# puzzlepaint/camera_calibration

Measured on NVIDIA H100. Metric: LM iterations/sec, higher is better.
Workload: dtype f64

## Files before the change

### camera_calibration_b200/build.py

```python
from __future__ import annotations

import os
import subprocess
import sys
from concurrent.futures import ThreadPoolExecutor

HERE = os.path.dirname(os.path.abspath(__file__))
CSRC = os.path.join(HERE, "csrc")
LIB = os.path.join(CSRC, "libb200ba.so")
SOURCES = ["ba_kernels.cu", "ba_host.cu", "ba_dense.cu"]
HEADERS = ["ba_common.h", "ba_device.cuh", "ba_kernels.h", os.path.join("..", "..", "include", "b200ba.h")]
NVCC = os.environ.get("NVCC", "/usr/local/cuda/bin/nvcc")
FLAGS = ["-gencode", "arch=compute_90a,code=sm_90a", "-lineinfo", "-O3", "-std=c++17", "-Xcompiler", "-fPIC",
         "-Xcompiler", "-fvisibility=hidden"]


def _stale() -> bool:
    if not os.path.exists(LIB):
        return True
    t = os.path.getmtime(LIB)
    for f in SOURCES + HEADERS:
        if os.path.getmtime(os.path.join(CSRC, f)) > t:
            return True
    return False


# ... 27 lines not shown
```

### camera_calibration_b200/csrc/ba_dense.cu

```cuda

#include <algorithm>
#include <cstdio>

#include "ba_kernels.h"
#include "ba_tile.cuh"

namespace b200ba {

namespace {

constexpr int BM = 128;
constexpr int LDT = BM + 4;
__host__ __device__ constexpr int gemm_threads(int bn) { return 4 * (bn / 32) * 32; }
constexpr size_t gemm_smem(int bn, int bk, int stages) {
  return static_cast<size_t>(stages) * bk * (LDT + bn + 4) * sizeof(double);
}

__device__ __forceinline__ void cp_async16(void* smem, const void* gmem, int src_bytes) {
  const unsigned s = static_cast<unsigned>(__cvta_generic_to_shared(smem));
  asm volatile("cp.async.cg.shared.global [%0], [%1], 16, %2;\n" ::"r"(s), "l"(gmem), "r"(src_bytes));
}
__device__ __forceinline__ void cp_async8(void* smem, const void* gmem, int src_bytes) {
  const unsigned s = static_cast<unsigned>(__cvta_generic_to_shared(smem));
  asm volatile("cp.async.ca.shared.global [%0], [%1], 8, %2;\n" ::"r"(s), "l"(gmem), "r"(src_bytes));
// ... 302 lines not shown
    configured_dev[dev & 63] = true;
  }
  potrf_trinv_tile_kernel<<<tile::CTAS, tile::THREADS, sizeof(tile::Shared), s>>>(Ain, lda_in, n, Lout, lda_out, Linv, info);
  return cudaGetLastError() == cudaSuccess ? 0 : 1;
}

__global__ void add_diagonal_map_kernel(int n, double* S, DenseMap map, double lambda) {
  const int c = blockIdx.x * blockDim.x + threadIdx.x;
  if (c < n) S[map.col_offset(c) + c] += lambda;
}
void launch_add_diagonal_map(int n, double* S, const DenseMap& map, double lambda, cudaStream_t s) {
  if (n > 0) add_diagonal_map_kernel<<<(n + 255) / 256, 256, 0, s>>>(n, S, map, lambda);
}

__global__ void trsv_store_tile_kernel(const double* __restrict__ Linv, const double* __restrict__ b, int live,
                                       double* __restrict__ out, bool transpose) {
  const int tid = threadIdx.x;
  if (tid >= live) return;
  double acc = 0.0;
  if (!transpose) {
    for (int c = 0; c <= tid; ++c) acc = fma(Linv[c * PT + tid], b[c], acc);
  } else {
    for (int i = tid; i < live; ++i) acc = fma(Linv[tid * PT + i], b[i], acc);
  }
  out[tid] = acc;
}

constexpr int TS2_THREADS = 256;
constexpr int TS2_LD = PT + 2;
constexpr size_t kTs2Smem = static_cast<size_t>(PT) * TS2_LD * sizeof(double);

__device__ __forceinline__ void stage_tile_async(double* dst, const double* __restrict__ src) {
  for (int ch = threadIdx.x; ch < PT * PT / 2; ch += TS2_THREADS) {
    const int c = ch >> 6, i2 = (ch & 63) * 2;
    cp_async16(dst + c * TS2_LD + i2, src + c * PT + i2, 16);
  }
  cp_async_commit();
}

// ... 35 lines not shown
      b_below[r] = v;
  }
  if (!chain) return;
  cp_async_wait<0>();
  __syncthreads();
  double s0 = 0.0, s1 = 0.0;
  for (int c = half; c <= row; c += 4) {
    s0 = fma(ts2_smem[c * TS2_LD + row], bs[c], s0);
    if (c + 2 <= row) s1 = fma(ts2_smem[(c + 2) * TS2_LD + row], bs[c + 2], s1);
  }
  part[half][row] = s0 + s1;
  __syncthreads();
  if (half == 0 && live_row) y_next[row] = part[0][row] + part[1][row];
}

__global__ void __launch_bounds__(TS2_THREADS, 1)
    trsv_backward2_kernel(const double* __restrict__ Lpack, const int64_t* __restrict__ panel_off,
                          const int* __restrict__ panel_h, int NB, int r0, int live, const double* __restrict__ x_t,
                          double* __restrict__ y , const double* __restrict__ Linv_prev,
                          double* __restrict__ x_prev ) {
  extern __shared__ __align__(16) double ts2_smem[];
  __shared__ double xs[PT], ysm[PT], part[2][PT];
  const int tid = threadIdx.x;
  const bool chain = blockIdx.x == 0;
  if (chain) stage_tile_async(ts2_smem, Linv_prev);
  if (tid < PT) xs[tid] = (tid < live) ? x_t[tid] : 0.0;
  __syncthreads();
  const int warp = tid >> 5, lane = tid & 31;
  const int cbase = r0 - PT * (static_cast<int>(blockIdx.x) + 1);
#pragma unroll
  for (int batch = 0; batch < 2; ++batch) {
    double l[8][4];
#pragma unroll
    for (int q = 0; q < 8; ++q) {
      const int c = cbase + warp * 16 + batch * 8 + q;
      const int k = c / NB;
      const double* col = Lpack + panel_off[k] + static_cast<int64_t>(c - k * NB) * panel_h[k] + (r0 - k * NB);
#pragma unroll
      for (int u = 0; u < 4; ++u) l[q][u] = (lane + 32 * u < live) ? col[lane + 32 * u] : 0.0;
    }
#pragma unroll
    for (int q = 0; q < 8; ++q) {
      double acc = 0.0;
#pragma unroll
      for (int u = 0; u < 4; ++u) acc = fma(l[q][u], xs[lane + 32 * u], acc);
#pragma unroll
      for (int o = 16; o > 0; o >>= 1) acc += __shfl_xor_sync(0xffffffffu, acc, o);
      if (lane == 0) {
        const int c = cbase + warp * 16 + batch * 8 + q;
        const double v = y[c] - acc;
        if (chain)
          ysm[c - cbase] = v;
        else
          y[c] = v;
      }
    }
  }
  if (!chain) return;
  cp_async_wait<0>();
  __syncthreads();
  const int j = tid & (PT - 1), half = tid >> 7;
  double s0 = 0.0, s1 = 0.0;
  const double* colj = ts2_smem + j * TS2_LD;
  for (int i = j + half; i < PT; i += 4) {
    s0 = fma(colj[i], ysm[i], s0);
    if (i + 2 < PT) s1 = fma(colj[i + 2], ysm[i + 2], s1);
  }
  part[half][j] = s0 + s1;
  __syncthreads();
  if (half == 0) x_prev[j] = part[0][j] + part[1][j];
}

int dense_plan(DenseCtx* d, int n, int nb, int rank, int ranks) {
  d->n = n;
  d->rank = rank;
  d->ranks = ranks;
  d->NB = nb;
  d->nblk = (n + nb - 1) / nb;
  d->ntiles = (n + PT - 1) / PT;
  d->map.nb = nb;
  d->map.ranks = ranks;
  d->map.blocks_per_rank = (d->nblk + ranks - 1) / ranks;
  d->map.ld = (n + 1) / 2 * 2;
  d->chunk = static_cast<int64_t>(d->map.blocks_per_rank) * nb * d->map.ld;
  d->panel_off.assign(d->nblk + 1, 0);
  d->panel_h.assign(std::max(1, d->nblk), 0);
  for (int k = 0; k < d->nblk; ++k) {
    const int hk = n - k * nb;
    d->panel_h[k] = (hk + 1) / 2 * 2;
    d->panel_off[k + 1] = d->panel_off[k] + static_cast<int64_t>(d->panel_h[k]) * nb + static_cast<int64_t>(nb / PT) * PT * PT;
  }
  return 0;
}

int dense_factor(DenseCtx* d) {
  const int n = d->n, NB = d->NB, R = d->ranks, me = d->rank;
  if (n == 0) return 0;
  const int sub_n = NB / PT;
  cudaStream_t sm = d->s_main, sp = d->s_panel;
  auto owner = [&](int k) { return k % R; };
  const bool use_aux = R == 1 && d->s_aux != nullptr;
  cudaEventRecord(d->ev_misc, sm);
  cudaStreamWaitEvent(sp, d->ev_misc, 0);

  auto update = [&](int k, int j_first, int j_last, cudaStream_t st, bool owned_only) -> int {
    if (j_first >= d->nblk || j_first > j_last) return 0;
    const int k0 = k * NB, kw = std::min(NB, n - k0);
    const int j0 = j_first * NB;
    const int jn = std::min(n, (std::min(j_last, d->nblk - 1) + 1) * NB) - j0;
    if (jn <= 0) return 0;
    GemmArgs g{};
    g.M = n - j0;
    g.N = jn;
    g.K = kw;
    g.A = d->Lpack + d->panel_off[k] + (j0 - k0);
    g.lda = d->panel_h[k];
    g.B = g.A;
    g.ldb = g.lda;
// ... 56 lines not shown
            u.ldb = hk;
            u.C = Sk_w + static_cast<int64_t>(c0 + PT) * ld + (c0 + PT);
            u.ldc = ld;
            u.alpha = -1.0;
            u.beta = 1.0;
            u.a_aligned = u.b_aligned = gemm_operand_aligned(u.A, u.lda);
            if (launch_dgemm_nt(u, true, false, sp, true)) return 1;
          }
        }
      }
    }
    if (R > 1) {
      if (d->bcast(P, static_cast<size_t>(hk) * NB + static_cast<size_t>(sub_n) * PT * PT, owner(k), sp, d->user)) return 1;
    }
    cudaEventRecord(d->ev_ready[k & 1], sp);
    cudaStreamWaitEvent(sm, d->ev_ready[k & 1], 0);
    if (k + 3 < d->nblk && update(k, k + 3, d->nblk - 1, sm, R > 1)) return 1;
    cudaEventRecord(d->ev_main[k & 1], sm);
    if (use_aux) {
      if (k >= 1) cudaStreamWaitEvent(sp, d->ev_half2[(k - 1) & 1], 0);
      if (k + 1 < d->nblk && update(k, k + 1, k + 1, sp, false)) return 1;
      if (k + 2 < d->nblk) {
        cudaStreamWaitEvent(d->s_aux, d->ev_ready[k & 1], 0);
        if (k > 0) cudaStreamWaitEvent(d->s_aux, d->ev_main[(k - 1) & 1], 0);
        if (update(k, k + 2, k + 2, d->s_aux, false)) return 1;
      }
      cudaEventRecord(d->ev_half2[k & 1], d->s_aux);
      continue;
    }
    if (k + 1 < d->nblk && owner(k + 1) == me && update(k, k + 1, k + 1, sp, false)) return 1;
    if (k + 2 < d->nblk && owner(k + 2) == me) {
      if (k > 0) cudaStreamWaitEvent(sp, d->ev_main[(k - 1) & 1], 0);
      if (update(k, k + 2, k + 2, sp, false)) return 1;
    }
  }
  if (use_aux && d->nblk >= 1) cudaStreamWaitEvent(sp, d->ev_half2[(d->nblk - 1) & 1], 0);
  cudaEventRecord(d->ev_misc, sp);
  cudaStreamWaitEvent(sm, d->ev_misc, 0);
  return cudaGetLastError() == cudaSuccess ? 0 : 1;
}

int dense_solve(DenseCtx* d, double* b) {
  const int n = d->n, NB = d->NB;
  if (n == 0) return 0;
  cudaStream_t sm = d->s_main;
  auto linv_of = [&](int t) {
    const int k = (t * PT) / NB, sub = (t * PT - k * NB) / PT;
    return d->Lpack + d->panel_off[k] + static_cast<int64_t>(d->panel_h[k]) * NB + static_cast<int64_t>(sub) * PT * PT;
  };
  static bool configured_dev[64] = {};
  int dev = 0;
  cudaGetDevice(&dev);
  if (!configured_dev[dev & 63]) {
    cudaFuncSetAttribute(trsv_forward2_kernel, cudaFuncAttributeMaxDynamicSharedMemorySize, static_cast<int>(kTs2Smem));
    cudaFuncSetAttribute(trsv_backward2_kernel, cudaFuncAttributeMaxDynamicSharedMemorySize, static_cast<int>(kTs2Smem));
    configured_dev[dev & 63] = true;
  }
  const int T = d->ntiles;
  trsv_store_tile_kernel<<<1, PT, 0, sm>>>(linv_of(0), b, std::min(PT, n), d->tmp, false);
  for (int t = 0; t + 1 < T; ++t) {
    const int c0 = t * PT, k = c0 / NB, off = c0 - k * NB;
    const int rows_below = n - c0 - PT;
    const double* Lp = d->Lpack + d->panel_off[k] + static_cast<int64_t>(off) * d->panel_h[k] + off + PT;
    trsv_forward2_kernel<<<(rows_below + PT - 1) / PT, TS2_THREADS, kTs2Smem, sm>>>(Lp, d->panel_h[k], rows_below, d->tmp + c0,
                                                                                    b + c0 + PT, linv_of(t + 1), d->tmp + c0 + PT);
  }
  {
    const int r0 = (T - 1) * PT;
    trsv_store_tile_kernel<<<1, PT, 0, sm>>>(linv_of(T - 1), d->tmp + r0, std::min(PT, n - r0), b + r0, true);
  }
  for (int t = T - 1; t >= 1; --t) {
    const int r0 = t * PT, live = std::min(PT, n - r0);
    trsv_backward2_kernel<<<r0 / PT, TS2_THREADS, kTs2Smem, sm>>>(d->Lpack, d->d_panel_off, d->d_panel_h, NB, r0, live, b + r0,
                                                                  d->tmp, linv_of(t - 1), b + r0 - PT);
  }
  return cudaGetLastError() == cudaSuccess ? 0 : 1;
}


constexpr int GV_ROWS = 128;
__global__ void gemv_t_stage1_kernel(int rows, int cols, int64_t ld, const double* __restrict__ B,
                                     const double* __restrict__ u, double* __restrict__ partial) {
  const int c = blockIdx.x * blockDim.x + threadIdx.x;
  const int r0 = blockIdx.y * GV_ROWS, r1 = min(rows, r0 + GV_ROWS);
  if (c >= cols) return;
  double a0 = 0.0, a1 = 0.0;
  int r = r0;
  for (; r + 1 < r1; r += 2) {
    a0 = fma(B[static_cast<int64_t>(r) * ld + c], u[r], a0);
    a1 = fma(B[static_cast<int64_t>(r + 1) * ld + c], u[r + 1], a1);
  }
  if (r < r1) a0 = fma(B[static_cast<int64_t>(r) * ld + c], u[r], a0);
  partial[static_cast<int64_t>(blockIdx.y) * cols + c] = a0 + a1;
// ... 42 lines not shown
```

### camera_calibration_b200/csrc/ba_host.cu

```cuda

#include <cublas_v2.h>
#include <cusolverDn.h>
#include <dlfcn.h>

#include <algorithm>
#include <cmath>
#include <cstdarg>
#include <cstdio>
#include <cstring>
#include <limits>
#include <string>
#include <vector>

#include "ba_kernels.h"

using namespace b200ba;

namespace {

std::string g_create_error;

struct NcclUniqueId {
  char internal[128];
};
// ... 124 lines not shown
  bool have_report = false;
  std::vector<int64_t> img_cam_groups;
  int* d_img_group_off = nullptr;
  uint32_t* d_img_group_obs = nullptr;
  bool have_images = false;

  void* comm = nullptr;
  int rank = 0, n_ranks = 1;

  bool own_dense = true;
  DenseCtx dn;
  int dense_planned_ranks = 0, dense_planned_n = -1;
  int dense_nb = 0;
  cudaStream_t panel_stream = nullptr;
  cudaStream_t aux_stream = nullptr;
  int* d_ident_cols = nullptr;
  double* d_gemv_partial = nullptr;

  b200ba_timings timings{};
  struct Pending {
    int phase;
    cudaEvent_t a, b;
    bool own_a = true;
  };
  std::vector<Pending> pending;
  std::vector<cudaEvent_t> event_pool;
};

namespace {

// ... 211 lines not shown
  if (rc != 0) {
    h->error = std::string("ncclBroadcast: ") + (g_nccl.GetErrorString ? g_nccl.GetErrorString(rc) : "error");
    return 1;
  }
  return 0;
}

cudaError_t dense_create(DenseCtx* d, bool own_streams) {
  cudaError_t e = cudaSuccess;
  if (own_streams) {
    int lo = 0, hi = 0;
    cudaDeviceGetStreamPriorityRange(&lo, &hi);
    e = cudaStreamCreateWithFlags(&d->s_main, cudaStreamNonBlocking);
    if (e == cudaSuccess) e = cudaStreamCreateWithPriority(&d->s_panel, cudaStreamNonBlocking, hi);
    if (e == cudaSuccess) e = cudaStreamCreateWithPriority(&d->s_aux, cudaStreamNonBlocking, hi);
  }
  for (cudaEvent_t* ev : {&d->ev_ready[0], &d->ev_ready[1], &d->ev_main[0], &d->ev_main[1], &d->ev_half2[0],
                          &d->ev_half2[1], &d->ev_misc})
    if (e == cudaSuccess && !*ev) e = cudaEventCreateWithFlags(ev, cudaEventDisableTiming);
  return e;
}
void dense_release(DenseCtx* d, bool own_streams) {
  for (cudaEvent_t ev : {d->ev_ready[0], d->ev_ready[1], d->ev_main[0], d->ev_main[1], d->ev_half2[0], d->ev_half2[1],
                         d->ev_misc})
    if (ev) cudaEventDestroy(ev);
  if (own_streams)
    for (cudaStream_t s : {d->s_main, d->s_panel, d->s_aux})
      if (s) cudaStreamDestroy(s);
}

int plan_dense(b200ba_handle* h) {
  if (!h->own_dense || !h->have_layout) return 0;
  const int nd = h->L.nd;
  if (h->dense_planned_n == nd && h->dense_planned_ranks == h->n_ranks) return 0;
  DenseCtx& d = h->dn;
  const int nb = h->dense_nb > 0 ? h->dense_nb : (h->n_ranks == 1 ? 512 : 256);
  dense_plan(&d, nd, nb, h->rank, h->n_ranks);
  if (dev_alloc(h, &h->d_S, static_cast<size_t>(std::max<int64_t>(1, d.chunk * h->n_ranks)))) return 1;
  d.S = h->d_S;
  if (dev_alloc(h, &d.Lpack, static_cast<size_t>(std::max<int64_t>(1, d.panel_off[d.nblk])))) return 1;
  if (dev_alloc(h, &d.tmp, std::max(1, nd))) return 1;
  if (dev_alloc(h, &d.d_panel_off, d.panel_off.size())) return 1;
  if (dev_alloc(h, &d.d_panel_h, d.panel_h.size())) return 1;
  CUDA_TRY(h, cudaMemcpy(d.d_panel_off, d.panel_off.data(), d.panel_off.size() * sizeof(int64_t), cudaMemcpyHostToDevice));
  CUDA_TRY(h, cudaMemcpy(d.d_panel_h, d.panel_h.data(), d.panel_h.size() * sizeof(int), cudaMemcpyHostToDevice));
  {
    std::vector<int> ident(std::max(1, nd));
    for (int i = 0; i < nd; ++i) ident[i] = i;
    if (dev_alloc(h, &h->d_ident_cols, ident.size())) return 1;
    CUDA_TRY(h, cudaMemcpy(h->d_ident_cols, ident.data(), ident.size() * sizeof(int), cudaMemcpyHostToDevice));
  }
  if (dev_alloc(h, &h->d_gemv_partial, static_cast<size_t>(gemv_t_partial_size(h->L.nbd, std::max(1, nd))))) return 1;
  CUDA_TRY(h, cudaMemset(h->d_S, 0, static_cast<size_t>(std::max<int64_t>(1, d.chunk * h->n_ranks)) * sizeof(double)));
  d.info = h->d_info;
  d.s_main = h->stream;
  d.s_panel = h->panel_stream;
  d.s_aux = h->aux_stream;
  CUDA_TRY(h, dense_create(&d, false));
  d.bcast = nccl_bcast_cb;
  d.user = h;
  h->dense_planned_n = nd;
  h->dense_planned_ranks = h->n_ranks;
  return 0;
}

int make_layout(b200ba_handle* h, const b200ba_options* opt) {
  if (opt->regularization_weight != 0) {
    static bool warned = false;
    if (!warned) fprintf(stderr, "[b200ba] regularization_weight is ignored (the term is disabled in the reference, joint_optimization.cc:299-305)\n");
    warned = true;
  }
  Layout L{};
// ... 490 lines not shown
    if (L.nbd > 0 && nd > 0) launch_gemv_t(L.nbd, nd, nd, h->sys.B, h->d_u, -1.0, h->d_x + L.nbd, h->d_gemv_partial, h->stream);
    h->timings.kernel_launches += 4;
  }
  if (h->capture_S && capture_reduced_system(h)) return 1;
  if (R > 1 && nd > 0) {
    ScopedPhase ph(h, PH_ALLREDUCE);
    const int rc = g_nccl.ReduceScatter(h->d_S, h->d_S + static_cast<size_t>(h->rank) * d.chunk, static_cast<size_t>(d.chunk),
                                        kNcclDouble, kNcclSum, h->comm, h->stream);
    if (rc != 0) {
      h->error = std::string("ncclReduceScatter: ") + (g_nccl.GetErrorString ? g_nccl.GetErrorString(rc) : "error");
      return 1;
    }
  }
  {
    ScopedPhase ph(h, PH_FACTOR);
    if (dense_factor(&d)) {
      if (h->error.empty()) h->error = "dense_factor: launch failed";
      return 1;
    }
    h->timings.factor_flops += static_cast<double>(nd) * nd * nd / 3.0;
    if (R > 1) {
      const int rc = g_nccl.AllReduce(h->d_info, h->d_info, 1, kNcclInt32, kNcclMax, h->comm, h->stream);
      if (rc != 0) {
        h->error = "ncclAllReduce (factorisation status) failed";
        return 1;
      }
    }
  }
  {
    ScopedPhase ph(h, PH_SOLVE);
    if (dense_solve(&d, h->d_x + L.nbd)) {
      h->error = "dense_solve: launch failed";
      return 1;
    }
    h->timings.kernel_launches += 4 * d.ntiles;
  }
  {
    ScopedPhase ph(h, PH_SCHUR);
    if (L.nbd > 0 && nd > 0)
      launch_gemv_n(L.nbd, nd, nd, h->sys.B, h->d_x + L.nbd, h->d_y, h->stream);
    else if (L.nbd > 0)
      CUDA_TRY(h, cudaMemsetAsync(h->d_y, 0, L.nbd * sizeof(double), h->stream));
    launch_block_backsub2(L.bs, L.nblocks, h->d_Linv, h->d_u, h->d_y, h->d_x, h->stream);
    h->timings.kernel_launches += 1;
  }
  CUDA_TRY(h, cudaMemcpyAsync(h->h_flags, h->d_info, sizeof(int), cudaMemcpyDeviceToHost, h->stream));
  CUDA_TRY(h, cudaMemcpyAsync(h->h_flags + 1, h->d_fail, sizeof(int), cudaMemcpyDeviceToHost, h->stream));
  if (sync_stream(h)) return 1;
  *spd = (h->h_flags[0] == 0 && h->h_flags[1] == 0) ? 1 : 0;
  return 0;
}

int check_ready(b200ba_handle* h, const b200ba_options* opt) {
  if (!h) return 1;
  if (!opt) {
    h->error = "options are NULL";
    return 2;
  }
  if (!h->have_state) {
    h->error = "no state: call b200ba_set_state first";
    return 2;
  }
  CUDA_TRY(h, cudaSetDevice(h->device));
// ... 17 lines not shown
  F(h->out_trial.residual); F(h->out_trial.cost);
  F(h->sys.base); F(h->d_W); F(h->d_S); F(h->d_Linv); F(h->d_v); F(h->d_y); F(h->d_x); F(h->d_potrf_work);
  F(h->d_info); F(h->d_fail); F(h->d_straggler_list); F(h->d_straggler_count); F(h->d_perm); F(h->d_lp_stage);
  F(h->d_group_of_block); F(h->d_group_blocks); F(h->d_flags); F(h->d_cols); F(h->d_count); F(h->d_Wc); F(h->d_P); F(h->d_u);
  F(h->d_contract);
  if (h->h_count) cudaFreeHost(h->h_count);
  h->h_count = nullptr;
  if (h->h_contract) cudaFreeHost(h->h_contract);
  h->h_contract = nullptr;
  F(h->d_partial); F(h->d_scal); F(h->d_rot);
  F(h->rep.err); F(h->rep.mag); F(h->rep.cam_off); F(h->rep.cell_off); F(h->rep.cell_order); F(h->rep.Q);
  F(h->rep.partial); F(h->rep.select_hist); F(h->rep.hist); F(h->rep.kl); F(h->rep.cams); F(h->d_rep_stage);
  h->have_report = false;
  F(h->d_img_group_off); F(h->d_img_group_obs);
  h->have_images = false;
  F(h->dn.Lpack); F(h->dn.tmp); F(h->dn.d_panel_off); F(h->dn.d_panel_h); F(h->d_ident_cols); F(h->d_gemv_partial);
  h->dn.S = nullptr;
  h->dense_planned_n = -1;
  if (h->h_scal) cudaFreeHost(h->h_scal);
  if (h->h_flags) cudaFreeHost(h->h_flags);
  h->h_scal = nullptr;
  h->h_flags = nullptr;
}

int setup_report(b200ba_handle* h) {
  if (h->have_report) return 0;
  const int64_t n = h->n_obs;
  const int nc = h->n_cameras;
  constexpr int kCells = kReportBiasCells * kReportBiasCells;
  std::vector<int64_t> cam_off(nc + 1, 0);
  for (int64_t o = 0; o < n; ++o) ++cam_off[h->h_obs_camera[o] + 1];
// ... 406 lines not shown
  }
  TRYC(dev_alloc(h, &h->d_lp_stage, n));
  if (n > 0) {
    h->h_obs_imageset.assign(p->obs_imageset, p->obs_imageset + n);
    h->h_obs_camera.assign(p->obs_camera, p->obs_camera + n);
    h->h_obs_point.assign(p->obs_point, p->obs_point + n);
    h->h_obs_xy.assign(p->obs_xy, p->obs_xy + 2 * n);
  }
  if (const char* e = getenv("B200BA_DENSE")) h->own_dense = !(strcmp(e, "lib") == 0 || strcmp(e, "0") == 0);
  if (const char* e = getenv("B200BA_DENSE_NB")) h->dense_nb = std::max(128, atoi(e) / 128 * 128);
  {
    int lo = 0, hi = 0;
    cudaDeviceGetStreamPriorityRange(&lo, &hi);
    TRYC(cuda_ok(cudaStreamCreateWithPriority(&h->panel_stream, cudaStreamNonBlocking, hi), "cudaStreamCreate"));
    TRYC(cuda_ok(cudaStreamCreateWithPriority(&h->aux_stream, cudaStreamNonBlocking, hi), "cudaStreamCreate"));
  }
  if (const char* e = getenv("B200BA_GROUPED")) h->force_grouped = atoi(e);
  h->pb.n_obs = n;
  h->pb.obs_imageset = h->d_obs_imageset;
  h->pb.obs_camera = h->d_obs_camera;
  h->pb.obs_point = h->d_obs_point;
  h->pb.obs_xy = h->d_obs_xy;
  for (int i = 0; i < 2; ++i) {
    TRYC(dev_alloc(h, &h->st[i].points, 3 * static_cast<size_t>(h->n_points)));
    TRYC(dev_alloc(h, &h->st[i].rig_tr_global, 7 * static_cast<size_t>(h->n_imagesets)));
    TRYC(dev_alloc(h, &h->st[i].camera_tr_rig, 7 * static_cast<size_t>(h->n_cameras)));
    TRYC(dev_alloc(h, &h->st[i].intrinsics, h->intr_total));
    TRYC(dev_alloc(h, &h->st[i].image_tr_global, 12 * static_cast<size_t>(h->n_imagesets) * h->n_cameras));
    TRYC(dev_alloc(h, &h->st[i].tangents, h->tan_total));
  }
// ... 19 lines not shown
  if (h->comm && g_nccl.CommDestroy) g_nccl.CommDestroy(h->comm);
  resolve_timings(h);
  for (auto e : h->event_pool) cudaEventDestroy(e);
  for (int i = 0; i < 2; ++i) {
    if (h->ev_syrk[i]) cudaEventDestroy(h->ev_syrk[i]);
    if (h->ev_scatter[i]) cudaEventDestroy(h->ev_scatter[i]);
  }
  if (h->ev_s_ready) cudaEventDestroy(h->ev_s_ready);
  free_handle_buffers(h);
  if (h->cublas) cublasDestroy(h->cublas);
  if (h->cusolver) cusolverDnDestroy(h->cusolver);
  if (h->stream) cudaStreamDestroy(h->stream);
  if (h->side_stream) cudaStreamDestroy(h->side_stream);
  if (h->panel_stream) cudaStreamDestroy(h->panel_stream);
  if (h->aux_stream) cudaStreamDestroy(h->aux_stream);
  dense_release(&h->dn, false);
  delete h;
}

int b200ba_set_state(b200ba_handle* h, const b200ba_state* s) {
  if (!h) return 1;
  if (!s || !s->points || !s->rig_tr_global || !s->camera_tr_rig || !s->intrinsics) {
    h->error = "NULL state array";
    return 2;
  }
  CUDA_TRY(h, cudaSetDevice(h->device));
  StateDev& d = h->st[h->cur];
  CUDA_TRY(h, cudaMemcpyAsync(d.points, s->points, 3 * sizeof(double) * h->n_points, cudaMemcpyHostToDevice, h->stream));
  CUDA_TRY(h, cudaMemcpyAsync(d.rig_tr_global, s->rig_tr_global, 7 * sizeof(double) * h->n_imagesets, cudaMemcpyHostToDevice, h->stream));
  CUDA_TRY(h, cudaMemcpyAsync(d.camera_tr_rig, s->camera_tr_rig, 7 * sizeof(double) * h->n_cameras, cudaMemcpyHostToDevice, h->stream));
// ... 722 lines not shown
  CallScope cs(&g_create_error);
  if (int rc = cs.use_device(device)) return rc;
  DenseCtx d;
  dense_plan(&d, n, nb, 0, 1);
  double* dA = nullptr;
  double* db = nullptr;
  cs.ok(dense_create(&d, true));
  cs.alloc(&dA, static_cast<size_t>(n) * n);
  cs.alloc(&d.S, static_cast<size_t>(d.chunk));
  cs.alloc(&d.Lpack, static_cast<size_t>(d.panel_off[d.nblk]));
  cs.alloc(&d.tmp, static_cast<size_t>(n));
  cs.alloc(&d.d_panel_off, d.panel_off.size());
  cs.alloc(&d.d_panel_h, d.panel_h.size());
  cs.alloc(&db, static_cast<size_t>(n));
  cs.alloc(&d.info, 1);
  if (cs.rc == 0) {
    cs.ok(cudaMemcpy(dA, A, static_cast<size_t>(n) * n * sizeof(double), cudaMemcpyHostToDevice));
    cs.ok(cudaMemcpy(db, b, static_cast<size_t>(n) * sizeof(double), cudaMemcpyHostToDevice));
    cs.ok(cudaMemcpy(d.d_panel_off, d.panel_off.data(), d.panel_off.size() * sizeof(int64_t), cudaMemcpyHostToDevice));
    cs.ok(cudaMemcpy(d.d_panel_h, d.panel_h.data(), d.panel_h.size() * sizeof(int), cudaMemcpyHostToDevice));
    cs.ok(cudaMemset(d.S, 0, static_cast<size_t>(d.chunk) * sizeof(double)));
    cs.ok(cudaMemset(d.info, 0, sizeof(int)));
    cs.ok(cudaMemcpy2D(d.S, d.map.ld * sizeof(double), dA, static_cast<size_t>(n) * sizeof(double),
                       static_cast<size_t>(n) * sizeof(double), n, cudaMemcpyDeviceToDevice));
    cs.ok(cudaDeviceSynchronize());
  }
  if (cs.rc == 0) {
    cs.record(0, d.s_main);
    if (dense_factor(&d)) cs.fail("b200ba_dense_cholesky_solve: kernel launch failed");
    cs.record(1, d.s_main);
    if (cs.rc == 0 && dense_solve(&d, db)) cs.fail("b200ba_dense_cholesky_solve: kernel launch failed");
    cs.record(2, d.s_main);
    cs.ok(cudaStreamSynchronize(d.s_main));
    cs.ok(cudaStreamSynchronize(d.s_panel));
  }
  if (cs.rc == 0) {
    if (factor_ms) *factor_ms = cs.elapsed_ms(0, 1);
    if (solve_ms) *solve_ms = cs.elapsed_ms(1, 2);
    int info = 0;
    cs.ok(cudaMemcpy(&info, d.info, sizeof(int), cudaMemcpyDeviceToHost));
    cs.ok(cudaMemcpy(x, db, static_cast<size_t>(n) * sizeof(double), cudaMemcpyDeviceToHost));
    if (cs.rc == 0 && info != 0) {
      g_create_error = "b200ba_dense_cholesky_solve: the matrix is not positive definite";
      cs.rc = 4;
    }
  }
  dense_release(&d, true);
  return cs.rc;
}

int b200ba_schur_solve(int device, int32_t bs, int32_t nb, int32_t nd, const double* D, const double* B,
                       const double* C, const double* b1, const double* b2, double* x) {
  if (bs < 1 || bs > 6 || nb < 0 || nd < 1 || !D || !B || !C || !b1 || !b2 || !x) {
    g_create_error = "b200ba_schur_solve: bad argument";
    return 2;
  }
// ... 1572 lines not shown
```

### camera_calibration_b200/csrc/ba_kernels.h

```cpp
#pragma once
#include <vector>

#include "ba_common.h"

namespace b200ba {

void launch_prepare_state(const ProblemDev& pb, const Layout& L, const StateDev& st, int64_t n_control_total,
                          cudaStream_t s);
void launch_residual_jacobian(int uniform_model, bool jac, const ProblemDev& pb, const Layout& L,
                              const StateDev& st, double2* last_projection, const ObsOut& out, double huber,
                              uint32_t* straggler_list, int* straggler_count, cudaStream_t s,
                              cudaEvent_t main_done = nullptr);
void launch_straggler_pass(int uniform_model, bool jac, const ProblemDev& pb, const Layout& L, const StateDev& st,
                           double2* last_projection, const ObsOut& out, double huber, uint32_t* straggler_list,
                           int* straggler_count, cudaStream_t s);
void launch_accumulate_list(const ProblemDev& pb, const Layout& L, const StateDev& st, const ObsOut& out,
                            const SystemDev& sys, double huber, const uint32_t* list, const int* count, cudaStream_t s);
void launch_expand_jacobian(const ProblemDev& pb, const Layout& L, const StateDev& st, const ObsOut& out, double* jac,
                            cudaStream_t s);
void set_main_eval_budget(int budget);
void launch_accumulate_scatter(const ProblemDev& pb, const Layout& L, const StateDev& st, const ObsOut& out,
                               const SystemDev& sys, double huber, cudaStream_t s);
void launch_accumulate_cells(const ProblemDev& pb, const Layout& L, const StateDev& st, const ObsOut& out,
                             const SystemDev& sys, double huber, cudaStream_t s);
// ... 143 lines not shown
void launch_add_diagonal_map(int n, double* S, const DenseMap& map, double lambda, cudaStream_t s);

struct DenseCtx {
  int n = 0, NB = 256, nblk = 0, ntiles = 0;
  int rank = 0, ranks = 1;
  DenseMap map{};
  int64_t chunk = 0;
  std::vector<int64_t> panel_off;
  std::vector<int> panel_h;
  double* S = nullptr;
  double* Lpack = nullptr;
  double* tmp = nullptr;
  int64_t* d_panel_off = nullptr;
  int* d_panel_h = nullptr;
  int* info = nullptr;
  cudaStream_t s_main = nullptr, s_panel = nullptr, s_aux = nullptr;
  cudaEvent_t ev_ready[2] = {nullptr, nullptr}, ev_main[2] = {nullptr, nullptr}, ev_half2[2] = {nullptr, nullptr}, ev_misc = nullptr;
  int (*bcast)(double* buf, size_t count, int root, cudaStream_t s, void* user) = nullptr;
  void* user = nullptr;
};
int dense_plan(DenseCtx* d, int n, int nb, int rank, int ranks);
int dense_factor(DenseCtx* d);
int dense_solve(DenseCtx* d, double* b);

}
```

Measured before the change: 24.36.

## Overlap forward TRSV with factorization and fuse backward sweep into persistent kernel

The forward triangular solve is launched on a new low-priority stream as each panel finishes, so it overlaps the Cholesky factorization instead of running afterwards. The backward sweep is replaced by a single cooperative persistent kernel in which CTAs own tiles and signal completion through epoch-tagged acquire/release flags, removing about one launch per tile. This removes per-tile launch overhead and serialization. In exchange it adds spin-wait polling with a timeout error path, extra stream synchronization, and possible contention between the forward sweep and the factorization.

```diff
diff --git a/camera_calibration_b200/build.py b/camera_calibration_b200/build.py
--- a/camera_calibration_b200/build.py
+++ b/camera_calibration_b200/build.py
@@ -9,7 +9,7 @@
 CSRC = os.path.join(HERE, "csrc")
 LIB = os.path.join(CSRC, "libb200ba.so")
 SOURCES = ["ba_kernels.cu", "ba_host.cu", "ba_dense.cu"]
-HEADERS = ["ba_common.h", "ba_device.cuh", "ba_kernels.h", os.path.join("..", "..", "include", "b200ba.h")]
+HEADERS = ["ba_common.h", "ba_device.cuh", "ba_kernels.h", "ba_tile.cuh", "ba_trsv.cuh", os.path.join("..", "..", "include", "b200ba.h")]
 NVCC = os.environ.get("NVCC", "/usr/local/cuda/bin/nvcc")
 FLAGS = ["-gencode", "arch=compute_90a,code=sm_90a", "-lineinfo", "-O3", "-std=c++17", "-Xcompiler", "-fPIC",
          "-Xcompiler", "-fvisibility=hidden"]
diff --git a/camera_calibration_b200/csrc/ba_dense.cu b/camera_calibration_b200/csrc/ba_dense.cu
--- a/camera_calibration_b200/csrc/ba_dense.cu
+++ b/camera_calibration_b200/csrc/ba_dense.cu
@@ -4,6 +4,7 @@
 
 #include "ba_kernels.h"
 #include "ba_tile.cuh"
+#include "ba_trsv.cuh"
 
 namespace b200ba {
 
@@ -340,15 +341,11 @@
 }
 
 __global__ void trsv_store_tile_kernel(const double* __restrict__ Linv, const double* __restrict__ b, int live,
-                                       double* __restrict__ out, bool transpose) {
+                                       double* __restrict__ out) {
   const int tid = threadIdx.x;
   if (tid >= live) return;
   double acc = 0.0;
-  if (!transpose) {
-    for (int c = 0; c <= tid; ++c) acc = fma(Linv[c * PT + tid], b[c], acc);
-  } else {
-    for (int i = tid; i < live; ++i) acc = fma(Linv[tid * PT + i], b[i], acc);
-  }
+  for (int c = 0; c <= tid; ++c) acc = fma(Linv[c * PT + tid], b[c], acc);
   out[tid] = acc;
 }
 
@@ -414,61 +411,84 @@
   if (half == 0 && live_row) y_next[row] = part[0][row] + part[1][row];
 }
 
-__global__ void __launch_bounds__(TS2_THREADS, 1)
-    trsv_backward2_kernel(const double* __restrict__ Lpack, const int64_t* __restrict__ panel_off,
-                          const int* __restrict__ panel_h, int NB, int r0, int live, const double* __restrict__ x_t,
-                          double* __restrict__ y , const double* __restrict__ Linv_prev,
-                          double* __restrict__ x_prev ) {
-  extern __shared__ __align__(16) double ts2_smem[];
-  __shared__ double xs[PT], ysm[PT], part[2][PT];
-  const int tid = threadIdx.x;
-  const bool chain = blockIdx.x == 0;
-  if (chain) stage_tile_async(ts2_smem, Linv_prev);
-  if (tid < PT) xs[tid] = (tid < live) ? x_t[tid] : 0.0;
-  __syncthreads();
-  const int warp = tid >> 5, lane = tid & 31;
-  const int cbase = r0 - PT * (static_cast<int>(blockIdx.x) + 1);
-#pragma unroll
-  for (int batch = 0; batch < 2; ++batch) {
-    double l[8][4];
-#pragma unroll
-    for (int q = 0; q < 8; ++q) {
-      const int c = cbase + warp * 16 + batch * 8 + q;
-      const int k = c / NB;
-      const double* col = Lpack + panel_off[k] + static_cast<int64_t>(c - k * NB) * panel_h[k] + (r0 - k * NB);
-#pragma unroll
-      for (int u = 0; u < 4; ++u) l[q][u] = (lane + 32 * u < live) ? col[lane + 32 * u] : 0.0;
-    }
-#pragma unroll
-    for (int q = 0; q < 8; ++q) {
-      double acc = 0.0;
-#pragma unroll
-      for (int u = 0; u < 4; ++u) acc = fma(l[q][u], xs[lane + 32 * u], acc);
+__device__ __forceinline__ unsigned ld_acquire_u32(const unsigned* p) {
+  unsigned v;
+  asm volatile("ld.acquire.gpu.global.u32 %0, [%1];\n" : "=r"(v) : "l"(p) : "memory");
+  return v;
+}
+__device__ __forceinline__ void st_release_u32(unsigned* p, unsigned v) {
+  asm volatile("st.release.gpu.global.u32 [%0], %1;\n" ::"l"(p), "r"(v) : "memory");
+}
+struct TrsvDeviceExec {
+  const trsv::Args& a;
+  trsv::Shared& sh;
+  trsv::Thread th;
+  template <class F>
+  __device__ __forceinline__ void run(F f) {
+    f(th, static_cast<int>(threadIdx.x));
+    __syncthreads();
+  }
+  __device__ __forceinline__ bool wait(int t) {
+    if (threadIdx.x == 0) {
+      int ok = 0;
+      unsigned ns = 32;
+      for (long long i = 0;; ++i) {
+        if (ld_acquire_u32(a.flags + t) == a.epoch) {
+          ok = 1;
+          break;
+        }
+        if (i >= trsv::kMaxPolls || *reinterpret_cast<volatile unsigned*>(a.err) == a.epoch) {
+          atomicExch(a.err, a.epoch);
+          break;
+        }
+        __nanosleep(ns);
+        if (ns < 256) ns *= 2;
+      }
+      sh.go = ok;
+    }
+    __syncthreads();
+    return sh.go != 0;
+  }
+  __device__ __forceinline__ void publish(int v) {
+    if (threadIdx.x == 0) {
+      __threadfence();
+      st_release_u32(a.flags + v, a.epoch);
+    }
+  }
+  __device__ __forceinline__ double load_x(const double* p) { return __ldcg(p); }
+  __device__ __forceinline__ void stage_linv(const double* __restrict__ src) {
+    for (int ch = threadIdx.x; ch < PT * PT / 2; ch += trsv::THREADS) {
+      const int c = ch >> 6, i2 = (ch & 63) * 2;
+      cp_async16(sh.linv + c * trsv::LINV_LD + i2, src + c * PT + i2, 16);
+    }
+    cp_async_commit();
+  }
+  __device__ __forceinline__ void wait_linv() {
+    cp_async_wait<0>();
+    __syncthreads();
+  }
+  __device__ __forceinline__ void apply(trsv::Shared& s, double* ys) {
+    const int warp = threadIdx.x >> 5, lane = threadIdx.x & 31;
+#pragma unroll
+    for (int q = 0; q < trsv::CPW; ++q) {
+      double acc = trsv::lane_partial(th.l[q], s.xs, lane);
 #pragma unroll
       for (int o = 16; o > 0; o >>= 1) acc += __shfl_xor_sync(0xffffffffu, acc, o);
       if (lane == 0) {
-        const int c = cbase + warp * 16 + batch * 8 + q;
-        const double v = y[c] - acc;
-        if (chain)
-          ysm[c - cbase] = v;
-        else
-          y[c] = v;
-      }
-    }
-  }
-  if (!chain) return;
-  cp_async_wait<0>();
-  __syncthreads();
-  const int j = tid & (PT - 1), half = tid >> 7;
-  double s0 = 0.0, s1 = 0.0;
-  const double* colj = ts2_smem + j * TS2_LD;
-  for (int i = j + half; i < PT; i += 4) {
-    s0 = fma(colj[i], ysm[i], s0);
-    if (i + 2 < PT) s1 = fma(colj[i + 2], ysm[i + 2], s1);
-  }
-  part[half][j] = s0 + s1;
-  __syncthreads();
-  if (half == 0) x_prev[j] = part[0][j] + part[1][j];
+        const int c = warp * trsv::CPW + q;
+        ys[c] = ys[c] - acc;
+      }
+    }
+    __syncthreads();
+  }
+};
+
+__global__ void __launch_bounds__(trsv::THREADS, 1) trsv_backward_kernel(trsv::Args a) {
+  extern __shared__ __align__(16) unsigned char trsv_smem[];
+  trsv::Shared& sh = *reinterpret_cast<trsv::Shared*>(trsv_smem);
+  double* ys = reinterpret_cast<double*>(trsv_smem + sizeof(trsv::Shared));
+  TrsvDeviceExec ex{a, sh, {}};
+  trsv::backward_program(ex, sh, ys, a, static_cast<int>(blockIdx.x), static_cast<int>(gridDim.x));
 }
 
 int dense_plan(DenseCtx* d, int n, int nb, int rank, int ranks) {
@@ -478,6 +498,7 @@
   d->NB = nb;
   d->nblk = (n + nb - 1) / nb;
   d->ntiles = (n + PT - 1) / PT;
+  d->trsv_grid = 0;
   d->map.nb = nb;
   d->map.ranks = ranks;
   d->map.blocks_per_rank = (d->nblk + ranks - 1) / ranks;
@@ -493,15 +514,43 @@
   return 0;
 }
 
-int dense_factor(DenseCtx* d) {
-  const int n = d->n, NB = d->NB, R = d->ranks, me = d->rank;
+static const double* linv_tile(const DenseCtx* d, int t) {
+  const int k = (t * PT) / d->NB, sub = (t * PT - k * d->NB) / PT;
+  return d->Lpack + d->panel_off[k] + static_cast<int64_t>(d->panel_h[k]) * d->NB + static_cast<int64_t>(sub) * PT * PT;
+}
+int dense_factor(DenseCtx* d, double* b) {
+  const int n = d->n, NB = d->NB, R = d->ranks, me = d->rank, T = d->ntiles;
   if (n == 0) return 0;
+  if (!d->s_fwd) return 1;
   const int sub_n = NB / PT;
-  cudaStream_t sm = d->s_main, sp = d->s_panel;
+  cudaStream_t sm = d->s_main, sp = d->s_panel, sf = d->s_fwd;
   auto owner = [&](int k) { return k % R; };
   const bool use_aux = R == 1 && d->s_aux != nullptr;
+  {
+    static bool configured_dev[64] = {};
+    int dev = 0;
+    cudaGetDevice(&dev);
+    if (!configured_dev[dev & 63]) {
+      cudaFuncSetAttribute(trsv_forward2_kernel, cudaFuncAttributeMaxDynamicSharedMemorySize, static_cast<int>(kTs2Smem));
+      configured_dev[dev & 63] = true;
+    }
+  }
   cudaEventRecord(d->ev_misc, sm);
   cudaStreamWaitEvent(sp, d->ev_misc, 0);
+  cudaStreamWaitEvent(sf, d->ev_misc, 0);
+
+  int t_fwd = 0;
+  auto forward = [&](int k) {
+    if (k == 0) trsv_store_tile_kernel<<<1, PT, 0, sf>>>(linv_tile(d, 0), b, std::min(PT, n), d->tmp);
+    const int covered = std::min(n, (k + 1) * NB);
+    for (; t_fwd + 1 < T && (t_fwd + 1) * PT < covered; ++t_fwd) {
+      const int c0 = t_fwd * PT, kt = c0 / NB, off = c0 - kt * NB;
+      const int rows_below = n - c0 - PT;
+      const double* Lp = d->Lpack + d->panel_off[kt] + static_cast<int64_t>(off) * d->panel_h[kt] + off + PT;
+      trsv_forward2_kernel<<<(rows_below + PT - 1) / PT, TS2_THREADS, kTs2Smem, sf>>>(
+          Lp, d->panel_h[kt], rows_below, d->tmp + c0, b + c0 + PT, linv_tile(d, t_fwd + 1), d->tmp + c0 + PT);
+    }
+  };
 
   auto update = [&](int k, int j_first, int j_last, cudaStream_t st, bool owned_only) -> int {
     if (j_first >= d->nblk || j_first > j_last) return 0;
@@ -588,6 +637,8 @@
       if (d->bcast(P, static_cast<size_t>(hk) * NB + static_cast<size_t>(sub_n) * PT * PT, owner(k), sp, d->user)) return 1;
     }
     cudaEventRecord(d->ev_ready[k & 1], sp);
+    cudaStreamWaitEvent(sf, d->ev_ready[k & 1], 0);
+    forward(k);
     cudaStreamWaitEvent(sm, d->ev_ready[k & 1], 0);
     if (k + 3 < d->nblk && update(k, k + 3, d->nblk - 1, sm, R > 1)) return 1;
     cudaEventRecord(d->ev_main[k & 1], sm);
@@ -611,46 +662,46 @@
   if (use_aux && d->nblk >= 1) cudaStreamWaitEvent(sp, d->ev_half2[(d->nblk - 1) & 1], 0);
   cudaEventRecord(d->ev_misc, sp);
   cudaStreamWaitEvent(sm, d->ev_misc, 0);
+  cudaEventRecord(d->ev_misc, sf);
+  cudaStreamWaitEvent(sm, d->ev_misc, 0);
   return cudaGetLastError() == cudaSuccess ? 0 : 1;
 }
 
 int dense_solve(DenseCtx* d, double* b) {
-  const int n = d->n, NB = d->NB;
+  const int n = d->n, T = d->ntiles;
   if (n == 0) return 0;
-  cudaStream_t sm = d->s_main;
-  auto linv_of = [&](int t) {
-    const int k = (t * PT) / NB, sub = (t * PT - k * NB) / PT;
-    return d->Lpack + d->panel_off[k] + static_cast<int64_t>(d->panel_h[k]) * NB + static_cast<int64_t>(sub) * PT * PT;
-  };
-  static bool configured_dev[64] = {};
-  int dev = 0;
-  cudaGetDevice(&dev);
-  if (!configured_dev[dev & 63]) {
-    cudaFuncSetAttribute(trsv_forward2_kernel, cudaFuncAttributeMaxDynamicSharedMemorySize, static_cast<int>(kTs2Smem));
-    cudaFuncSetAttribute(trsv_backward2_kernel, cudaFuncAttributeMaxDynamicSharedMemorySize, static_cast<int>(kTs2Smem));
-    configured_dev[dev & 63] = true;
-  }
-  const int T = d->ntiles;
-  trsv_store_tile_kernel<<<1, PT, 0, sm>>>(linv_of(0), b, std::min(PT, n), d->tmp, false);
-  for (int t = 0; t + 1 < T; ++t) {
-    const int c0 = t * PT, k = c0 / NB, off = c0 - k * NB;
-    const int rows_below = n - c0 - PT;
-    const double* Lp = d->Lpack + d->panel_off[k] + static_cast<int64_t>(off) * d->panel_h[k] + off + PT;
-    trsv_forward2_kernel<<<(rows_below + PT - 1) / PT, TS2_THREADS, kTs2Smem, sm>>>(Lp, d->panel_h[k], rows_below, d->tmp + c0,
-                                                                                    b + c0 + PT, linv_of(t + 1), d->tmp + c0 + PT);
-  }
-  {
-    const int r0 = (T - 1) * PT;
-    trsv_store_tile_kernel<<<1, PT, 0, sm>>>(linv_of(T - 1), d->tmp + r0, std::min(PT, n - r0), b + r0, true);
-  }
-  for (int t = T - 1; t >= 1; --t) {
-    const int r0 = t * PT, live = std::min(PT, n - r0);
-    trsv_backward2_kernel<<<r0 / PT, TS2_THREADS, kTs2Smem, sm>>>(d->Lpack, d->d_panel_off, d->d_panel_h, NB, r0, live, b + r0,
-                                                                  d->tmp, linv_of(t - 1), b + r0 - PT);
-  }
+  if (!d->trsv_flags) return 1;
+  if (d->trsv_grid == 0) {
+    int dev = 0, sms = 0, per_sm = 0;
+    cudaGetDevice(&dev);
+    cudaDeviceGetAttribute(&sms, cudaDevAttrMultiProcessorCount, dev);
+    if (sms < 1) return 1;
+    const size_t smem = trsv::shared_bytes((T + sms - 1) / sms);
+    if (cudaFuncSetAttribute(trsv_backward_kernel, cudaFuncAttributeMaxDynamicSharedMemorySize, static_cast<int>(smem)) != cudaSuccess ||
+        cudaOccupancyMaxActiveBlocksPerMultiprocessor(&per_sm, trsv_backward_kernel, trsv::THREADS, smem) != cudaSuccess || per_sm < 1)
+      return 1;
+    d->trsv_grid = std::min(T, per_sm * sms);
+    d->trsv_smem = smem;
+  }
+  if (++d->trsv_epoch == 0) ++d->trsv_epoch;
+  trsv::Args a{};
+  a.Lpack = d->Lpack;
+  a.panel_off = d->d_panel_off;
+  a.panel_h = d->d_panel_h;
+  a.NB = d->NB;
+  a.n = n;
+  a.T = T;
+  a.y = d->tmp;
+  a.x = b;
+  a.flags = d->trsv_flags;
+  a.epoch = d->trsv_epoch;
+  a.err = d->trsv_flags + T;
+  void* args[] = {&a};
+  if (cudaLaunchCooperativeKernel(reinterpret_cast<const void*>(trsv_backward_kernel), dim3(d->trsv_grid), dim3(trsv::THREADS), args,
+                                  d->trsv_smem, d->s_main) != cudaSuccess)
+    return 1;
   return cudaGetLastError() == cudaSuccess ? 0 : 1;
 }
-
 
 constexpr int GV_ROWS = 128;
 __global__ void gemv_t_stage1_kernel(int rows, int cols, int64_t ld, const double* __restrict__ B,
diff --git a/camera_calibration_b200/csrc/ba_host.cu b/camera_calibration_b200/csrc/ba_host.cu
--- a/camera_calibration_b200/csrc/ba_host.cu
+++ b/camera_calibration_b200/csrc/ba_host.cu
@@ -162,6 +162,7 @@
   int dense_nb = 0;
   cudaStream_t panel_stream = nullptr;
   cudaStream_t aux_stream = nullptr;
+  cudaStream_t fwd_stream = nullptr;
   int* d_ident_cols = nullptr;
   double* d_gemv_partial = nullptr;
 
@@ -403,6 +404,7 @@
     e = cudaStreamCreateWithFlags(&d->s_main, cudaStreamNonBlocking);
     if (e == cudaSuccess) e = cudaStreamCreateWithPriority(&d->s_panel, cudaStreamNonBlocking, hi);
     if (e == cudaSuccess) e = cudaStreamCreateWithPriority(&d->s_aux, cudaStreamNonBlocking, hi);
+    if (e == cudaSuccess) e = cudaStreamCreateWithPriority(&d->s_fwd, cudaStreamNonBlocking, lo);
   }
   for (cudaEvent_t* ev : {&d->ev_ready[0], &d->ev_ready[1], &d->ev_main[0], &d->ev_main[1], &d->ev_half2[0],
                           &d->ev_half2[1], &d->ev_misc})
@@ -414,7 +416,7 @@
                          d->ev_misc})
     if (ev) cudaEventDestroy(ev);
   if (own_streams)
-    for (cudaStream_t s : {d->s_main, d->s_panel, d->s_aux})
+    for (cudaStream_t s : {d->s_main, d->s_panel, d->s_aux, d->s_fwd})
       if (s) cudaStreamDestroy(s);
 }
 
@@ -431,6 +433,8 @@
   if (dev_alloc(h, &d.tmp, std::max(1, nd))) return 1;
   if (dev_alloc(h, &d.d_panel_off, d.panel_off.size())) return 1;
   if (dev_alloc(h, &d.d_panel_h, d.panel_h.size())) return 1;
+  if (dev_alloc(h, &d.trsv_flags, static_cast<size_t>(d.ntiles) + 1)) return 1;
+  CUDA_TRY(h, cudaMemset(d.trsv_flags, 0, (static_cast<size_t>(d.ntiles) + 1) * sizeof(unsigned)));
   CUDA_TRY(h, cudaMemcpy(d.d_panel_off, d.panel_off.data(), d.panel_off.size() * sizeof(int64_t), cudaMemcpyHostToDevice));
   CUDA_TRY(h, cudaMemcpy(d.d_panel_h, d.panel_h.data(), d.panel_h.size() * sizeof(int), cudaMemcpyHostToDevice));
   {
@@ -445,6 +449,7 @@
   d.s_main = h->stream;
   d.s_panel = h->panel_stream;
   d.s_aux = h->aux_stream;
+  d.s_fwd = h->fwd_stream;
   CUDA_TRY(h, dense_create(&d, false));
   d.bcast = nccl_bcast_cb;
   d.user = h;
@@ -965,7 +970,7 @@
   }
   {
     ScopedPhase ph(h, PH_FACTOR);
-    if (dense_factor(&d)) {
+    if (dense_factor(&d, h->d_x + L.nbd)) {
       if (h->error.empty()) h->error = "dense_factor: launch failed";
       return 1;
     }
@@ -984,7 +989,7 @@
       h->error = "dense_solve: launch failed";
       return 1;
     }
-    h->timings.kernel_launches += 4 * d.ntiles;
+    h->timings.kernel_launches += d.ntiles + 1;
   }
   {
     ScopedPhase ph(h, PH_SCHUR);
@@ -997,7 +1002,13 @@
   }
   CUDA_TRY(h, cudaMemcpyAsync(h->h_flags, h->d_info, sizeof(int), cudaMemcpyDeviceToHost, h->stream));
   CUDA_TRY(h, cudaMemcpyAsync(h->h_flags + 1, h->d_fail, sizeof(int), cudaMemcpyDeviceToHost, h->stream));
+  if (nd > 0)
+    CUDA_TRY(h, cudaMemcpyAsync(h->h_flags + 2, d.trsv_flags + d.ntiles, sizeof(unsigned), cudaMemcpyDeviceToHost, h->stream));
   if (sync_stream(h)) return 1;
+  if (nd > 0 && dense_solve_failed(d, static_cast<unsigned>(h->h_flags[2]))) {
+    h->error = "dense_solve: the backward sweep gave up waiting for a tile";
+    return 1;
+  }
   *spd = (h->h_flags[0] == 0 && h->h_flags[1] == 0) ? 1 : 0;
   return 0;
 }
@@ -1045,7 +1056,7 @@
   h->have_report = false;
   F(h->d_img_group_off); F(h->d_img_group_obs);
   h->have_images = false;
-  F(h->dn.Lpack); F(h->dn.tmp); F(h->dn.d_panel_off); F(h->dn.d_panel_h); F(h->d_ident_cols); F(h->d_gemv_partial);
+  F(h->dn.Lpack); F(h->dn.tmp); F(h->dn.d_panel_off); F(h->dn.d_panel_h); F(h->dn.trsv_flags); F(h->d_ident_cols); F(h->d_gemv_partial);
   h->dn.S = nullptr;
   h->dense_planned_n = -1;
   if (h->h_scal) cudaFreeHost(h->h_scal);
@@ -1482,6 +1493,7 @@
     cudaDeviceGetStreamPriorityRange(&lo, &hi);
     TRYC(cuda_ok(cudaStreamCreateWithPriority(&h->panel_stream, cudaStreamNonBlocking, hi), "cudaStreamCreate"));
     TRYC(cuda_ok(cudaStreamCreateWithPriority(&h->aux_stream, cudaStreamNonBlocking, hi), "cudaStreamCreate"));
+    TRYC(cuda_ok(cudaStreamCreateWithPriority(&h->fwd_stream, cudaStreamNonBlocking, lo), "cudaStreamCreate"));
   }
   if (const char* e = getenv("B200BA_GROUPED")) h->force_grouped = atoi(e);
   h->pb.n_obs = n;
@@ -1531,6 +1543,7 @@
   if (h->side_stream) cudaStreamDestroy(h->side_stream);
   if (h->panel_stream) cudaStreamDestroy(h->panel_stream);
   if (h->aux_stream) cudaStreamDestroy(h->aux_stream);
+  if (h->fwd_stream) cudaStreamDestroy(h->fwd_stream);
   dense_release(&h->dn, false);
   delete h;
 }
@@ -2283,6 +2296,7 @@
   cs.alloc(&d.d_panel_h, d.panel_h.size());
   cs.alloc(&db, static_cast<size_t>(n));
   cs.alloc(&d.info, 1);
+  cs.alloc(&d.trsv_flags, static_cast<size_t>(d.ntiles) + 1);
   if (cs.rc == 0) {
     cs.ok(cudaMemcpy(dA, A, static_cast<size_t>(n) * n * sizeof(double), cudaMemcpyHostToDevice));
     cs.ok(cudaMemcpy(db, b, static_cast<size_t>(n) * sizeof(double), cudaMemcpyHostToDevice));
@@ -2290,13 +2304,14 @@
     cs.ok(cudaMemcpy(d.d_panel_h, d.panel_h.data(), d.panel_h.size() * sizeof(int), cudaMemcpyHostToDevice));
     cs.ok(cudaMemset(d.S, 0, static_cast<size_t>(d.chunk) * sizeof(double)));
     cs.ok(cudaMemset(d.info, 0, sizeof(int)));
+    cs.ok(cudaMemset(d.trsv_flags, 0, (static_cast<size_t>(d.ntiles) + 1) * sizeof(unsigned)));
     cs.ok(cudaMemcpy2D(d.S, d.map.ld * sizeof(double), dA, static_cast<size_t>(n) * sizeof(double),
                        static_cast<size_t>(n) * sizeof(double), n, cudaMemcpyDeviceToDevice));
     cs.ok(cudaDeviceSynchronize());
   }
   if (cs.rc == 0) {
     cs.record(0, d.s_main);
-    if (dense_factor(&d)) cs.fail("b200ba_dense_cholesky_solve: kernel launch failed");
+    if (dense_factor(&d, db)) cs.fail("b200ba_dense_cholesky_solve: kernel launch failed");
     cs.record(1, d.s_main);
     if (cs.rc == 0 && dense_solve(&d, db)) cs.fail("b200ba_dense_cholesky_solve: kernel launch failed");
     cs.record(2, d.s_main);
@@ -2307,8 +2322,11 @@
     if (factor_ms) *factor_ms = cs.elapsed_ms(0, 1);
     if (solve_ms) *solve_ms = cs.elapsed_ms(1, 2);
     int info = 0;
+    unsigned sweep_err = 0;
     cs.ok(cudaMemcpy(&info, d.info, sizeof(int), cudaMemcpyDeviceToHost));
+    cs.ok(cudaMemcpy(&sweep_err, d.trsv_flags + d.ntiles, sizeof(unsigned), cudaMemcpyDeviceToHost));
     cs.ok(cudaMemcpy(x, db, static_cast<size_t>(n) * sizeof(double), cudaMemcpyDeviceToHost));
+    if (cs.rc == 0 && dense_solve_failed(d, sweep_err)) cs.fail("b200ba_dense_cholesky_solve: the backward sweep gave up waiting for a tile");
     if (cs.rc == 0 && info != 0) {
       g_create_error = "b200ba_dense_cholesky_solve: the matrix is not positive definite";
       cs.rc = 4;
diff --git a/camera_calibration_b200/csrc/ba_kernels.h b/camera_calibration_b200/csrc/ba_kernels.h
--- a/camera_calibration_b200/csrc/ba_kernels.h
+++ b/camera_calibration_b200/csrc/ba_kernels.h
@@ -181,13 +181,19 @@
   int64_t* d_panel_off = nullptr;
   int* d_panel_h = nullptr;
   int* info = nullptr;
+  unsigned* trsv_flags = nullptr;
+  unsigned trsv_epoch = 0;
+  int trsv_grid = 0;
+  size_t trsv_smem = 0;
   cudaStream_t s_main = nullptr, s_panel = nullptr, s_aux = nullptr;
+  cudaStream_t s_fwd = nullptr;
   cudaEvent_t ev_ready[2] = {nullptr, nullptr}, ev_main[2] = {nullptr, nullptr}, ev_half2[2] = {nullptr, nullptr}, ev_misc = nullptr;
   int (*bcast)(double* buf, size_t count, int root, cudaStream_t s, void* user) = nullptr;
   void* user = nullptr;
 };
 int dense_plan(DenseCtx* d, int n, int nb, int rank, int ranks);
-int dense_factor(DenseCtx* d);
+int dense_factor(DenseCtx* d, double* b);
 int dense_solve(DenseCtx* d, double* b);
+inline bool dense_solve_failed(const DenseCtx& d, unsigned err_word) { return d.trsv_epoch != 0 && err_word == d.trsv_epoch; }
 
 }
diff --git a/camera_calibration_b200/csrc/ba_trsv.cuh b/camera_calibration_b200/csrc/ba_trsv.cuh
--- /dev/null
+++ b/camera_calibration_b200/csrc/ba_trsv.cuh
@@ -0,0 +1,138 @@
+#pragma once
+
+#include <cmath>
+#include <cstdint>
+
+#if defined(__CUDACC__)
+#define B200_TRSV_HD __host__ __device__ __forceinline__
+#else
+#define B200_TRSV_HD inline
+#endif
+
+namespace b200ba {
+namespace trsv {
+
+constexpr int PT = 128;
+constexpr int THREADS = 512;
+constexpr int WARPS = THREADS / 32;
+constexpr int CPW = PT / WARPS;
+constexpr int LINV_LD = PT + 2;
+constexpr long long kMaxPolls = 1ll << 22;
+
+struct Args {
+  const double* Lpack;
+  const int64_t* panel_off;
+  const int* panel_h;
+  int NB, n, T;
+  const double* y;
+  double* x;
+  unsigned* flags;
+  unsigned epoch;
+  unsigned* err;
+};
+
+struct alignas(16) Shared {
+  double linv[PT * LINV_LD];
+  double xs[PT];
+  double part[2][PT];
+  int go;
+};
+inline size_t shared_bytes(int owned) { return sizeof(Shared) + static_cast<size_t>(owned) * PT * sizeof(double); }
+
+struct Thread {
+  double l[CPW][4];
+};
+
+B200_TRSV_HD const double* column(const Args& a, int c, int r0) {
+  const int k = c / a.NB;
+  return a.Lpack + a.panel_off[k] + static_cast<int64_t>(c - k * a.NB) * a.panel_h[k] + (r0 - k * a.NB);
+}
+B200_TRSV_HD const double* linv_of(const Args& a, int t) {
+  const int k = (t * PT) / a.NB, sub = (t * PT - k * a.NB) / PT;
+  return a.Lpack + a.panel_off[k] + static_cast<int64_t>(a.panel_h[k]) * a.NB + static_cast<int64_t>(sub) * PT * PT;
+}
+
+B200_TRSV_HD void load_block(Thread& th, const Args& a, int c0, int r0, int tid, int live) {
+  const int warp = tid >> 5, lane = tid & 31;
+#pragma unroll
+  for (int q = 0; q < CPW; ++q) {
+    const double* col = column(a, c0 + warp * CPW + q, r0);
+#pragma unroll
+    for (int u = 0; u < 4; ++u) th.l[q][u] = (lane + 32 * u < live) ? col[lane + 32 * u] : 0.0;
+  }
+}
+B200_TRSV_HD double lane_partial(const double (&l)[4], const double* xs, int lane) {
+  double acc = 0.0;
+#pragma unroll
+  for (int u = 0; u < 4; ++u) acc = fma(l[u], xs[lane + 32 * u], acc);
+  return acc;
+}
+B200_TRSV_HD double finish_half(const double* linv, const double* ys, int j, int half) {
+  double s0 = 0.0, s1 = 0.0;
+  const double* colj = linv + j * LINV_LD;
+  for (int i = j + half; i < PT; i += 4) {
+    s0 = fma(colj[i], ys[i], s0);
+    if (i + 2 < PT) s1 = fma(colj[i + 2], ys[i + 2], s1);
+  }
+  return s0 + s1;
+}
+B200_TRSV_HD double last_tile(const double* linv, const double* ys, int j, int live) {
+  double acc = 0.0;
+  for (int i = j; i < live; ++i) acc = fma(linv[j * PT + i], ys[i], acc);
+  return acc;
+}
+
+template <class Ex>
+B200_TRSV_HD void backward_program(Ex& ex, Shared& sh, double* ys, const Args& a, int cta, int G) {
+  const int T = a.T, n = a.n;
+  if (cta >= T) return;
+  const int owned = (T - 1 - cta) / G + 1;
+  auto tile_of = [&](int s) { return cta + s * G; };
+  ex.run([&](Thread&, int tid) {
+    for (int s = 0; s < owned; ++s)
+      for (int r = tid; r < PT; r += THREADS) {
+        const int row = tile_of(s) * PT + r;
+        ys[s * PT + r] = row < n ? a.y[row] : 0.0;
+      }
+  });
+  int fin = owned - 1;
+  if (tile_of(fin) == T - 1) {
+    const int r0 = (T - 1) * PT, live = n - r0;
+    const double* linv = linv_of(a, T - 1);
+    ex.run([&](Thread&, int tid) {
+      if (tid < live) a.x[r0 + tid] = last_tile(linv, ys + fin * PT, tid, live);
+    });
+    ex.publish(T - 1);
+    --fin;
+  }
+  if (fin >= 0) ex.stage_linv(linv_of(a, tile_of(fin)));
+  for (int t = T - 1; t >= 1 && fin >= 0; --t) {
+    const int r0 = t * PT, live = n - r0 < PT ? n - r0 : PT;
+    const int first = fin;
+    ex.run([&](Thread& th, int tid) { load_block(th, a, tile_of(first) * PT, r0, tid, live); });
+    if (!ex.wait(t)) return;
+    ex.run([&](Thread&, int tid) {
+      if (tid < PT) sh.xs[tid] = tid < live ? ex.load_x(a.x + r0 + tid) : 0.0;
+    });
+    for (int s = first; s >= 0; --s) {
+      const int v = tile_of(s);
+      if (s != first) ex.run([&](Thread& th, int tid) { load_block(th, a, v * PT, r0, tid, live); });
+      ex.apply(sh, ys + s * PT);
+      if (v == t - 1) {
+        ex.wait_linv();
+        ex.run([&](Thread&, int tid) {
+          if (tid < 2 * PT) sh.part[tid >> 7][tid & (PT - 1)] = finish_half(sh.linv, ys + s * PT, tid & (PT - 1), tid >> 7);
+        });
+        ex.run([&](Thread&, int tid) {
+          if (tid < PT) a.x[v * PT + tid] = sh.part[0][tid] + sh.part[1][tid];
+        });
+        ex.publish(v);
+        --fin;
+        if (fin >= 0) ex.stage_linv(linv_of(a, tile_of(fin)));
+      }
+    }
+  }
+}
+
+}
+}
```

After: 24.90, median of 6. +2.2%, better.
